# DanielPS555/Radix-sort-Merge-Sort-CUDA---Lab-y-practicos-GPGPU-2023

Measured on AMD Instinct MI355X. Metric: Mkeys/s sorting uint32, n=2^28, 1 GPU (+ merge-sort at 2/4/8), higher is better.
Workload: dtype u32; 1 GPU; LSD radix sort (8-bit digits, onesweep), n=2^28 uint32 u32, device-resident (BASELINE config 3); n_per_gpu=268435456, algo=radix, key=u32, dist=u32, parallelism=single GPU

## Files before the change

radix-sort-merge-sort-cuda---lab-y-practicos-gpgpu-2023_amd/csrc/fin_block.h:

```cpp
#pragma once
#include "segsort.h"

#include "devutil.h"

namespace labsort {

namespace {

#ifndef LABSORT_FIN_PREFETCH
#define LABSORT_FIN_PREFETCH 1
#endif

__device__ __forceinline__ uint32_t wave_incl_scan_dpp(uint32_t x) {
    x += (uint32_t)__builtin_amdgcn_update_dpp(0, (int)x, 0x111, 0xf, 0xf, false);
    x += (uint32_t)__builtin_amdgcn_update_dpp(0, (int)x, 0x112, 0xf, 0xf, false);
    x += (uint32_t)__builtin_amdgcn_update_dpp(0, (int)x, 0x114, 0xf, 0xf, false);
    x += (uint32_t)__builtin_amdgcn_update_dpp(0, (int)x, 0x118, 0xf, 0xf, false);
    x += (uint32_t)__builtin_amdgcn_update_dpp(0, (int)x, 0x142, 0xa, 0xf, false);
    x += (uint32_t)__builtin_amdgcn_update_dpp(0, (int)x, 0x143, 0xc, 0xf, false);
    return x;
}

template <int BLOCK, int KPT>
struct FinSmem {
    static constexpr int R = 256, W = BLOCK / WAVE, TILE = BLOCK * KPT;
    static_assert(TILE <= 65536, "16-bit LDS slots");
    static_assert(W == 4, "the fold holds one counter row per wave in registers");
    uint32_t keys[TILE];
    alignas(16) uint32_t cnt[W * R];
    alignas(16) uint32_t offs[W * R];
    uint32_t probe[WAVE];
    uint32_t ordered;
};

struct FinStripe {
    size_t sb;
    uint32_t ws0;
    uint32_t nf;
    uint32_t ng;
    bool tail_ok;
};
template <int W, int KPT>
__device__ __forceinline__ FinStripe fin_stripe(uint32_t b, uint32_t len, uint32_t lane, uint32_t wid) {
    if (len > (uint32_t)(W * WAVE * KPT)) len = 0u;
    const uint32_t jn = (len + (uint32_t)(W * WAVE) - 1u) / (uint32_t)(W * WAVE);
    const uint32_t ws0 = wid * jn * WAVE;
    const uint32_t rem = ws0 < len ? len - ws0 : 0u;
    const uint32_t nf = min(jn, rem / WAVE);
    const uint32_t tail = nf < jn ? rem - nf * WAVE : 0u;
    return {(size_t)b + ws0, ws0, nf, nf + (tail ? 1u : 0u), lane < tail};
}

template <int KPT>
__device__ __forceinline__ void fin_load(const uint32_t *in, const FinStripe &g, uint32_t lane, uint32_t (&k)[KPT]) {
    const char *pb = reinterpret_cast<const char *>(in + g.sb);
    const uint32_t lb = lane * 4u;
    if (g.nf == (uint32_t)KPT) {
#pragma unroll
        for (int j = 0; j < KPT; ++j) k[j] = ld_stream<NT_TILE>(reinterpret_cast<const uint32_t *>(pb + (lb + (uint32_t)(j * WAVE * 4))));
    } else {
#pragma unroll
        for (int j = 0; j < KPT; ++j) {
            k[j] = 0xFFFFFFFFu;
            if ((uint32_t)j < g.nf || ((uint32_t)j == g.nf && g.tail_ok))
                k[j] = ld_stream<NT_TILE>(reinterpret_cast<const uint32_t *>(pb + (lb + (uint32_t)(j * WAVE * 4))));
        }
    }
}

template <int BLOCK, int KPT>
__device__ __forceinline__ void fin_pass(FinSmem<BLOCK, KPT> &sm, const uint32_t (&k)[KPT], uint32_t shift, uint32_t ng,
                                         bool atomic_rank, uint32_t lane, uint32_t wid) {
    constexpr int W = FinSmem<BLOCK, KPT>::W, R = FinSmem<BLOCK, KPT>::R;
    uint32_t *wh = sm.cnt + wid * R;
    uint32_t *wo = sm.offs + wid * R;
    uint32_t n0 = ng, n1 = ng;
    asm volatile("" : "+s"(n0), "+s"(n1));
    uint32_t z = 0u;
    asm volatile("" : "+v"(z));
    *reinterpret_cast<uint4 *>(wh + 4u * lane) = make_uint4(z, z, z, z);
    uint32_t rank[KPT / 2] = {};
#pragma unroll
    for (int j = 0; j < KPT; ++j) {
        uint32_t r = 0u;
        if ((uint32_t)j < n0) r = rank8(wh, (k[j] >> shift) & 0xFFu, lane, atomic_rank);
        set16(rank, j, r);
    }
    __syncthreads();
    {
        uint4 c[W];
#pragma unroll
        for (int w = 0; w < W; ++w) c[w] = *reinterpret_cast<const uint4 *>(sm.cnt + w * R + 4u * lane);
        uint32_t tot[4] = {0u, 0u, 0u, 0u}, bef[4] = {0u, 0u, 0u, 0u};
#pragma unroll
        for (int w = 0; w < W; ++w) {
            const uint32_t cw[4] = {c[w].x, c[w].y, c[w].z, c[w].w};
            const bool before = (uint32_t)w < wid;
#pragma unroll
            for (int q = 0; q < 4; ++q) {
                tot[q] += cw[q];
                bef[q] += before ? cw[q] : 0u;
            }
        }
        const uint32_t s = tot[0] + tot[1] + tot[2] + tot[3];
        uint32_t run = wave_incl_scan_dpp(s) - s;
        uint4 o4;
        o4.x = run + bef[0];
        run += tot[0];
        o4.y = run + bef[1];
        run += tot[1];
        o4.z = run + bef[2];
        run += tot[2];
        o4.w = run + bef[3];
        *reinterpret_cast<uint4 *>(wo + 4u * lane) = o4;
    }
    __builtin_amdgcn_wave_barrier();
#pragma unroll
    for (int j = 0; j < KPT; ++j)
        if ((uint32_t)j < n1) set16(rank, j, wo[(k[j] >> shift) & 0xFFu] + get16(rank, j));
#pragma unroll
    for (int j = 0; j < KPT; ++j)
        if ((uint32_t)j < n1) sm.keys[get16(rank, j)] = k[j];
    __syncthreads();
}

template <int BLOCK, int KPT, int WPE>
__global__ __launch_bounds__(BLOCK, WPE) void k_fin_block(uint32_t *out, const uint32_t *__restrict__ off,
                                                           const uint32_t *__restrict__ hdr,
                                                           const uint32_t *__restrict__ list, HySel hy) {
    using S = FinSmem<BLOCK, KPT>;
    constexpr int W = S::W;
    constexpr int CLS = 3;
    constexpr bool PREFETCH = LABSORT_FIN_PREFETCH != 0;
    __shared__ S sm;
    if (hy.plan->hybrid == 0u) return;
    const uint32_t *in = hy.buf[hy.plan->fin_src];
    if (ld_agent(hdr) != 0u) return;
    const uint32_t cnt = hdr[SEG_HDR_CNT + CLS];
    const uint32_t tid = threadIdx.x, lane = tid & 63u, wid = __builtin_amdgcn_readfirstlane(tid >> 6);
    if (blockIdx.x >= cnt) return;
    probe_lane_order(sm.probe, &sm.ordered, lane, wid);
    __syncthreads();
    const bool atomic_rank = lane_order_probed(&sm.ordered);
    uint32_t nb, ne;
    {
        const uint32_t seg = __builtin_amdgcn_readfirstlane(list[blockIdx.x]);
        nb = __builtin_amdgcn_readfirstlane(off[seg]);
        ne = __builtin_amdgcn_readfirstlane(off[seg + 1]);
    }
    uint32_t k[KPT];
    FinStripe g = fin_stripe<W, KPT>(nb, ne - nb, lane, wid);
    if constexpr (PREFETCH) fin_load(in, g, lane, k);
    for (uint32_t it = blockIdx.x; it < cnt; it += gridDim.x) {
        if constexpr (!PREFETCH) {
            g = fin_stripe<W, KPT>(nb, ne - nb, lane, wid);
            fin_load(in, g, lane, k);
        }
        const bool more = it + gridDim.x < cnt;
        if (more) {
            const uint32_t seg = __builtin_amdgcn_readfirstlane(list[it + gridDim.x]);
            nb = __builtin_amdgcn_readfirstlane(off[seg]);
            ne = __builtin_amdgcn_readfirstlane(off[seg + 1]);
        }
        fin_pass(sm, k, 0u, g.ng, atomic_rank, lane, wid);
        {
            uint32_t n2 = g.ng;
            asm volatile("" : "+s"(n2));
#pragma unroll
            for (int j = 0; j < KPT; ++j)
                if ((uint32_t)j < n2) k[j] = sm.keys[g.ws0 + (uint32_t)j * WAVE + lane];
        }
        fin_pass(sm, k, 8u, g.ng, atomic_rank, lane, wid);
        FinStripe gn = g;
        uint32_t kn[PREFETCH ? KPT : 1];
        if constexpr (PREFETCH) {
            gn = fin_stripe<W, KPT>(nb, more ? ne - nb : 0u, lane, wid);
            fin_load(in, gn, lane, kn);
        }
        uint32_t nfs = g.nf;
        asm volatile("" : "+s"(nfs));
        const uint32_t *sk = sm.keys + g.ws0 + lane;
        char *ob = reinterpret_cast<char *>(out + g.sb);
        const uint32_t lb = lane * 4u;
        if (nfs == (uint32_t)KPT) {
#pragma unroll
            for (int j = 0; j < KPT; ++j) *reinterpret_cast<uint32_t *>(ob + (lb + (uint32_t)(j * WAVE * 4))) = sk[j * WAVE];
        } else {
#pragma unroll
            for (int j = 0; j < KPT; ++j)
                if ((uint32_t)j < nfs || ((uint32_t)j == nfs && g.tail_ok))
                    *reinterpret_cast<uint32_t *>(ob + (lb + (uint32_t)(j * WAVE * 4))) = sk[j * WAVE];
        }
        if constexpr (PREFETCH) {
            g = gn;
#pragma unroll
            for (int j = 0; j < KPT; ++j) k[j] = kn[j];
        }
    }
}

}

}
```

radix-sort-merge-sort-cuda---lab-y-practicos-gpgpu-2023_amd/csrc/kernels.hip:

```cpp
#include "common.h"
#include "devutil.h"
#include "host.h"
#include "lds_pass.h"

#include <cstdlib>
#include <cstring>
#include <type_traits>

namespace labsort {

__device__ __forceinline__ uint64_t mix64(uint64_t z) {
    z += 0x9E3779B97F4A7C15ull;
    z = (z ^ (z >> 30)) * 0xBF58476D1CE4E5B9ull;
    z = (z ^ (z >> 27)) * 0x94D049BB133111EBull;
    return z ^ (z >> 31);
}

__global__ __launch_bounds__(256) void k_fill(uint32_t *__restrict__ out, size_t n, uint64_t seed, int dist,
                                              uint64_t param, uint64_t first) {
    const size_t stride = (size_t)gridDim.x * blockDim.x;
    for (size_t i = (size_t)blockIdx.x * blockDim.x + threadIdx.x; i < n; i += stride) {
        const uint64_t gi = first + i;
        const uint64_t z = mix64(seed ^ (gi * 0x9E3779B97F4A7C15ull));
        const uint32_t hi = (uint32_t)(z >> 32);
// ... 162 lines not shown
                const bool s4 = fv(k[4 * u + 3]) == fa && fv(k[4 * u + 1]) == fa && fv(k[4 * u + 2]) == fa;
                if (s4) {
                    atomicAdd(ctr(fa), 4u);
                } else {
#pragma unroll
                    for (int j = 4 * u; j < 4 * u + 4; ++j) atomicAdd(ctr(fv(k[j])), 1u);
                }
            }
        };
        auto top = [&](uint32_t x) { return HY ? x >> (32 - HY_TOP_BITS) : fld(x, 2); };
        if (__ballot(top(k[0]) == top(k[3])) == 0ull) {
#pragma unroll
            for (int p = 0; p < NJ; ++p)
#pragma unroll
                for (int j = 0; j < 16; ++j) atomicAdd(&hj[p * JF + fld(k[j], p)], 1u);
            if constexpr (HY) {
#pragma unroll
                for (int j = 0; j < 16; ++j) atomicAdd(&ht[top(k[j])], 1u);
            }
            return;
        }
#pragma unroll
        for (int p = 0; p < NJ; ++p)
            add_field([&](uint32_t x) { return fld(x, p); }, [&](uint32_t f) { return &hj[p * JF + f]; });
        if constexpr (HY) add_field(top, [&](uint32_t f) { return &ht[f]; });
    };
    const uint32_t seg = blockIdx.x / bps, part = blockIdx.x % bps;
    const size_t sb = seg_start(seg, n), se = seg_start(seg + 1, n);
    const size_t per = (se - sb + bps - 1) / bps;
    const size_t beg = sb + (size_t)part * per < se ? sb + (size_t)part * per : se;
    const size_t end = beg + per < se ? beg + per : se;
    if ((((uintptr_t)keys) & 15u) == 0) {
        const size_t abeg = (beg + 3) & ~(size_t)3;
        const size_t vbeg = abeg < end ? abeg : end;
        for (size_t t = beg + threadIdx.x; t < vbeg; t += HIST_BLOCK) count(keys[t]);
        const size_t nv = (end - vbeg) / 4;
        const uint4 *v = reinterpret_cast<const uint4 *>(keys + vbeg);
        size_t i = threadIdx.x;
        uint4 c[4], x[4];
        if (i + 3 * HIST_BLOCK < nv) {
#pragma unroll
            for (int u = 0; u < 4; ++u) c[u] = ld_stream4<NT_HIST>(v + i + u * HIST_BLOCK);
        }
        for (; i + 3 * HIST_BLOCK < nv; i += 4 * HIST_BLOCK) {
            if (i + 7 * HIST_BLOCK < nv) {
#pragma unroll
                for (int u = 0; u < 4; ++u) x[u] = ld_stream4<NT_HIST>(v + i + (4 + u) * HIST_BLOCK);
            }
            count16(c);
#pragma unroll
            for (int u = 0; u < 4; ++u) c[u] = x[u];
        }
        for (; i < nv; i += HIST_BLOCK) {
            const uint4 x = ld_stream4<NT_HIST>(v + i);
            count(x.x); count(x.y); count(x.z); count(x.w);
        }
        for (size_t r = vbeg + nv * 4 + threadIdx.x; r < end; r += HIST_BLOCK) count(keys[r]);
    } else {
        for (size_t t = beg + threadIdx.x; t < end; t += HIST_BLOCK) count(keys[t]);
    }
    __syncthreads();
    for (int i = threadIdx.x; i < 256; i += HIST_BLOCK) {
        uint32_t c = 0;
#pragma unroll 8
        for (int q = 0; q < SL; ++q) c += h[i * SL + ((q + i) & (SL - 1))];
        if (c) atomicAdd(&hps[seg * 256 + i], c);
        if constexpr (HY) {
            uint32_t c2 = 0;
#pragma unroll
            for (int q = 0; q < 16; ++q) c2 += hj[JF + i * 16 + ((q + i) & 15)];
            if (c2) atomicAdd(&hy.hps2[seg * 256 + i], c2);
        }
    }
    const uint32_t rot = (blockIdx.x * (uint32_t)HIST_BLOCK) % ((uint32_t)NJ * JF);
    for (int i0 = threadIdx.x; i0 < NJ * JF; i0 += HIST_BLOCK) {
        int i = i0 + (int)rot;
        i = i >= NJ * JF ? i - NJ * JF : i;
        const uint32_t c = hj[i];
        const uint32_t p = (uint32_t)i / JF, f = (uint32_t)i % JF;
        if (c) atomicAdd(&joint[((p + 1) * NSEG + (f & 15u)) * 256 + (f >> 4)], c);
    }
    if constexpr (HY) {
        const uint32_t rot4 = (blockIdx.x * 272u) % (uint32_t)JF;
        for (uint32_t g0 = threadIdx.x; g0 < (uint32_t)JF; g0 += HIST_BLOCK) {
            const uint32_t f = (g0 + rot4) % (uint32_t)JF;
            uint32_t sum = 0;
#pragma unroll
            for (uint32_t q = 0; q < 4u; ++q) {
                const uint32_t c = ht[4u * f + q];
                sum += c;
                if (c) atomicAdd(&hy.top14[4u * f + q], c);
            }
            if (sum) atomicAdd(&joint[(3u * NSEG + (f & 15u)) * 256 + (f >> 4)], sum);
        }
    }
}

__device__ void build_segplan(SegPlan *__restrict__ sp, const uint32_t *__restrict__ hs, const uint32_t *start,
                              uint32_t mode, uint32_t *sh ) {
    const uint32_t t = threadIdx.x;
    uint32_t tot = 0;
    for (int s = 0; s < NSEG; ++s) {
        const uint32_t v = hs[s * 256 + t];
        sh[s * 256 + t] = v;
        tot += v;
    }
    uint32_t run = block_excl_scan<256, 256>(tot, sh + NSEG * 256);
    for (int s = 0; s < NSEG; ++s) {
        sp->base[s * 256 + t] = run;
        run += sh[s * 256 + t];
    }
    if (t <= (uint32_t)NSEG) sp->start[t] = start[t];
    if (t == 0) {
        uint32_t tp = 0, mx = 0;
        for (int s = 0; s <= NSEG; ++s) {
            sp->tpre[s] = tp;
            if (s < NSEG) {
                const uint32_t a0 = start[s] - start[s] % (uint32_t)OSP_TILE;
                const uint32_t ts = start[s + 1] > start[s] ? (start[s + 1] - a0 + OSP_TILE - 1) / OSP_TILE : 0u;
                tp += ts;
                mx = ts > mx ? ts : mx;
            }
        }
        sp->maxt = mx;
        sp->mode = mode;
        sp->segbits = mode == 2u ? 0u : 4u;
    }
}

__device__ void build_segplan_later(SegPlan *__restrict__ out, int q, uint32_t prev, uint32_t n, int seg_later,
                                    const uint32_t *hist, const uint32_t *__restrict__ joint, uint32_t *sh,
                                    uint32_t *start) {
    const uint32_t t = threadIdx.x;
    if (seg_later <= 0 || prev + 1u != (uint32_t)q) {
        for (int s = 0; s < NSEG; ++s) sh[s * 256 + t] = s ? 0u : hist[q * 256 + t];
        if (t <= (uint32_t)NSEG) start[t] = t ? n : 0u;
        __syncthreads();
        build_segplan(out, sh, start, 2u, sh);
        return;
    }
    const uint32_t ex = block_excl_scan<256, 256>(hist[prev * 256 + t], sh + NSEG * 256);
    if ((t & 15u) == 0) start[t >> 4] = ex;
    if (t == 0) start[NSEG] = n;
    __syncthreads();
    build_segplan(out, joint + (size_t)q * NSEG * 256, start, 1u, sh);
}

__global__ __launch_bounds__(256) void k_plan8(const uint32_t *__restrict__ hps, const uint32_t *__restrict__ joint,
                                               uint32_t n, int in_is_out, int seg_later, Plan *__restrict__ plan,
                                               SegPlan *__restrict__ sps, uint32_t *__restrict__ hist_out,
                                               uint4 *__restrict__ zp, size_t zn4, HyCounts hy) {
    constexpr uint32_t PW = 4;
    if (blockIdx.x >= PW) {
        const size_t stride = (size_t)(gridDim.x - PW) * blockDim.x;
        for (size_t i = (size_t)(blockIdx.x - PW) * blockDim.x + threadIdx.x; i < zn4; i += stride)
            zp[i] = make_uint4(0u, 0u, 0u, 0u);
        return;
    }
    const int me = (int)blockIdx.x;
    __shared__ uint32_t hist[4 * 256];
    __shared__ uint32_t sh[NSEG * 256 + 8];
    __shared__ uint32_t triv[4];
    __shared__ uint32_t start[NSEG + 1];
    __shared__ uint32_t prevs[4];
    __shared__ int first;
    __shared__ uint32_t max14;
    const uint32_t t = threadIdx.x;
    if (t < 4) triv[t] = 0;
    if (t == 0) max14 = 0u;
    __syncthreads();
    const uint32_t verdict = hy.ctl ? hy.ctl[HY_CTL_VERDICT] : 0u;
    if (hy.top14 && verdict == 0u) {
        uint32_t m = 0;
        for (uint32_t i = t; i < (uint32_t)HY_TOP; i += 256u) m = max(m, hy.top14[i]);
        atomicMax(&max14, m);
    }
    uint32_t v[4] = {0, 0, 0, 0};
    for (int s = 0; s < NSEG; ++s) {
        v[0] += hps[s * 256 + t];
#pragma unroll
        for (int p = 1; p < 4; ++p) v[p] += joint[(p * NSEG + s) * 256 + t];
    }
#pragma unroll
    for (int p = 0; p < 4; ++p) {
        hist[p * 256 + t] = v[p];
        if (me == 0) hist_out[p * 256 + t] = v[p];
        if (v[p] == n) triv[p] = 1;
    }
    if (t <= (uint32_t)NSEG) start[t] = seg_later < 0 ? (t ? n : 0u) : seg_start(t, n);
    __syncthreads();
    const bool hybrid = verdict ? verdict == HY_VERDICT_HYBRID
                                : hy.top14 && !triv[0] && !triv[1] && max14 <= min(hy.limit, HY_MAX_BUCKET);
    __syncthreads();
    if (hybrid && t < 2) triv[t] = 1;
    __syncthreads();
    if (t == 0 && me != 0) {
        int k = 0, last = -1;
        for (int p = 0; p < 4; ++p) {
            prevs[p] = NEXT_NONE;
            if (!triv[p]) {
                if (last >= 0) prevs[p] = (uint32_t)last;
                last = p;
                if (!k++) first = p;
            }
        }
        if (!k) first = -1;
    }
    if (t == 0 && me == 0) {
        int act[4];
        int k = 0;
        for (int p = 0; p < MAX_PASSES; ++p) {
            plan->src[p] = SEL_SKIP;
            plan->dst[p] = SEL_SKIP;
            plan->next[p] = NEXT_NONE;
            plan->prev[p] = NEXT_NONE;
        }
        for (int p = 0; p < 4; ++p) {
            prevs[p] = NEXT_NONE;
            if (!triv[p]) act[k++] = p;
        }
        for (int i = 0; i + 1 < k; ++i) {
            plan->next[act[i]] = (uint32_t)act[i + 1];
            plan->prev[act[i + 1]] = prevs[act[i + 1]] = (uint32_t)act[i];
        }
        plan->active = (uint32_t)k;
        first = k ? act[0] : -1;
        plan->hybrid = hybrid ? 1u : 0u;
        plan->fin_src = SEL_OUT;
        if (!hybrid) {
            plan_buffers(plan, act, k, in_is_out);
        } else {
            uint32_t src = SEL_IN;
            for (int i = 0; i < k; ++i) {
                plan->src[act[i]] = src;
                plan->dst[act[i]] = src = (i == k - 1 && !(k == 1 && in_is_out)) ? SEL_OUT : SEL_TMP;
            }
            plan->fin_src = src;
            plan->copy_from = SEL_SKIP;
        }
    }
    __syncthreads();
    if (first < 0 || me < first) return;
    if (me != first) {
        if (prevs[me] != NEXT_NONE)
            build_segplan_later(sps + me, me, prevs[me], n, seg_later, hist, joint, sh, start);
        return;
    }
    const uint32_t *hp = first == 0 ? hps : (hybrid && first == 2) ? hy.hps2 : nullptr;
    if (seg_later < 0 || !hp) {
        if (t <= (uint32_t)NSEG) start[t] = t ? n : 0u;
        for (int s = 0; s < NSEG; ++s) sh[s * 256 + t] = s ? 0u : hist[first * 256 + t];
        __syncthreads();
        build_segplan(sps + first, sh, start, 2u, sh);
    } else {
        for (int s = 0; s < NSEG; ++s) sh[s * 256 + t] = hp[s * 256 + t];
        __syncthreads();
        build_segplan(sps + first, sh, start, 0u, sh);
    }
}

__global__ __launch_bounds__(256) void k_final_copy(Bufs b, const Plan *__restrict__ plan, size_t n) {
    const uint32_t from = plan->copy_from;
    if (from == SEL_SKIP) return;
    const uint32_t *__restrict__ src = b.p[from];
    uint32_t *__restrict__ dst = b.p[SEL_OUT];
    const size_t stride = (size_t)gridDim.x * blockDim.x;
    const size_t tid = (size_t)blockIdx.x * blockDim.x + threadIdx.x;
    if (((((uintptr_t)src) | ((uintptr_t)dst)) & 15u) == 0) {
        const size_t nv = n / 4;
        for (size_t i = tid; i < nv; i += stride)
            reinterpret_cast<uint4 *>(dst)[i] = reinterpret_cast<const uint4 *>(src)[i];
        for (size_t i = nv * 4 + tid; i < n; i += stride) dst[i] = src[i];
    } else {
        for (size_t i = tid; i < n; i += stride) dst[i] = src[i];
    }
}

__device__ __forceinline__ uint32_t osp_pad(uint32_t i) { return i + (i >> 5); }

template <int BITS, int BLOCK, int KPT>
struct OsSmem {
    static constexpr int R = 1 << BITS, W = BLOCK / WAVE, TILE = BLOCK * KPT;
    uint32_t keys[TILE + TILE / 32];
    uint32_t whist[W * R];
    uint32_t gscan[R];
    uint32_t dstart[R];
    uint32_t delta[R];
    uint32_t wsum0[W];
    uint32_t wsum1[W];
    uint32_t tile;
};

template <int BITS, int BLOCK, int KPT>
__global__ __launch_bounds__(BLOCK) void k_onesweep(Bufs bufs, const Plan *__restrict__ plan, int pass, uint32_t n,
                                                    uint32_t flip, const uint32_t *__restrict__ ghist,
                                                    uint32_t *lookback, uint32_t *counter, uint32_t *err) {
    using S = OsSmem<BITS, BLOCK, KPT>;
    constexpr int R = S::R, W = S::W, TILE = S::TILE;
    constexpr uint32_t RM = R - 1;
    static_assert(R <= BLOCK, "one thread per digit");
    __shared__ S sm;

    const uint32_t srcsel = plan->src[pass];
    if (srcsel == SEL_SKIP) return;
    const uint32_t *__restrict__ in = bufs.p[srcsel];
    uint32_t *__restrict__ out = bufs.p[plan->dst[pass]];
    const uint32_t tid = threadIdx.x, lane = tid & 63u, wid = tid >> 6;
    const uint32_t shift = (uint32_t)pass * BITS;
// ... 1149 lines not shown
```

radix-sort-merge-sort-cuda---lab-y-practicos-gpgpu-2023_amd/csrc/segsort.hip:

```cpp
#include "segsort.h"

#include <algorithm>

#include "devutil.h"
#include "fin_block.h"
#include "host.h"
#include "seg_kernels.h"

namespace labsort {

namespace {

constexpr int BIN_BLOCK = 1024, BIN_SPT = 4;

__global__ __launch_bounds__(BIN_BLOCK) void k_seg_bin(const uint32_t *__restrict__ off, uint32_t nseg, uint32_t n,
                                                        uint32_t max_len, SegEdges e, uint32_t copy1,
                                                        uint32_t *__restrict__ hdr, uint32_t *__restrict__ lists,
                                                        size_t stride, const Plan *__restrict__ hyplan) {
    __shared__ uint32_t cnt[SEG_CLASSES], base[SEG_CLASSES];
    if (hyplan && hyplan->hybrid == 0u) return;
    const uint32_t tid = threadIdx.x, lane = tid & 63u;
    if (tid < (uint32_t)SEG_CLASSES) cnt[tid] = 0u;
    __syncthreads();
    uint32_t cls[BIN_SPT], pos[BIN_SPT];
    bool bad = false;
#pragma unroll
    for (int j = 0; j < BIN_SPT; ++j) {
        const uint32_t seg = blockIdx.x * (uint32_t)(BIN_BLOCK * BIN_SPT) + (uint32_t)j * BIN_BLOCK + tid;
        uint32_t c = SEG_CLASSES;
        if (seg < nseg) {
            const uint32_t a = off[seg], b = off[seg + 1];
            if (b < a || b > n) {
                bad = true;
            } else {
                const uint32_t len = b - a;
                if (max_len && len > max_len) bad = true;
                if (len > 1u || (len == 1u && copy1)) {
                    c = 0u;
#pragma unroll
                    for (int q = 0; q < SEG_CLASSES - 1; ++q) c += len > e.e[q] ? 1u : 0u;
                }
            }
            if (seg == 0u && a != 0u) bad = true;
            if (seg == nseg - 1u && b != n) bad = true;
        }
        cls[j] = c;
        pos[j] = 0u;
        if (lists) {
#pragma unroll
            for (uint32_t cc = 0; cc < (uint32_t)SEG_CLASSES; ++cc) {
                const uint64_t m = __ballot(c == cc);
                if (m == 0ull) continue;
                const uint32_t leader = (uint32_t)__ffsll((long long)m) - 1u;
                uint32_t wb = 0u;
                if (lane == leader) wb = atomicAdd(&cnt[cc], (uint32_t)__popcll(m));
                wb = __shfl(wb, (int)leader);
                if (c == cc) pos[j] = wb + mbcnt64(m);
            }
        }
    }
    if (bad) atomicOr(hdr, 1u);
    if (!lists) return;
    __syncthreads();
    if (tid < (uint32_t)SEG_CLASSES) base[tid] = cnt[tid] ? atomicAdd(hdr + SEG_HDR_CNT + tid, cnt[tid]) : 0u;
    __syncthreads();
#pragma unroll
    for (int j = 0; j < BIN_SPT; ++j) {
        const uint32_t seg = blockIdx.x * (uint32_t)(BIN_BLOCK * BIN_SPT) + (uint32_t)j * BIN_BLOCK + tid;
        if (cls[j] < (uint32_t)SEG_CLASSES) lists[(size_t)cls[j] * stride + base[cls[j]] + pos[j]] = seg;
    }
}

__global__ __launch_bounds__(256) void k_seg_ids(const uint32_t *__restrict__ off, uint32_t nseg, uint32_t n,
                                                 const uint32_t *__restrict__ idx, uint32_t *__restrict__ ids,
                                                 uint32_t *__restrict__ iota, const uint32_t *__restrict__ hdr) {
    if (ld_agent(hdr) != 0u) return;
    const size_t stride = (size_t)gridDim.x * blockDim.x;
    for (size_t i = (size_t)blockIdx.x * blockDim.x + threadIdx.x; i < n; i += stride) {
        if (iota) iota[i] = (uint32_t)i;
        if (!ids) continue;
        uint32_t p = idx ? idx[i] : (uint32_t)i;
        if (p >= n) p = n - 1u;
        uint32_t lo = 1u, hi = nseg;
        while (lo < hi) {
            const uint32_t mid = lo + (hi - lo) / 2u;
            if (off[mid] > p) hi = mid;
            else lo = mid + 1u;
        }
        ids[i] = lo - 1u;
    }
}

__global__ __launch_bounds__(256) void k_seg_gather(const uint32_t *__restrict__ src, const uint32_t *__restrict__ vsrc,
                                                    const uint32_t *__restrict__ perm, uint32_t *__restrict__ out,
                                                    uint32_t *__restrict__ vout, uint32_t n,
                                                    const uint32_t *__restrict__ hdr) {
    if (ld_agent(hdr) != 0u) return;
    const size_t stride = (size_t)gridDim.x * blockDim.x;
    for (size_t i = (size_t)blockIdx.x * blockDim.x + threadIdx.x; i < n; i += stride) {
        uint32_t p = perm ? perm[i] : (uint32_t)i;
        if (p >= n) p = n - 1u;
        out[i] = src[p];
        if (vsrc) vout[i] = vsrc[p];
    }
}

__global__ void k_seg_err_acc(uint32_t *hdr, uint32_t *inner) {
    if (threadIdx.x == 0 && blockIdx.x == 0) {
        if (*inner) hdr[SEG_HDR_DEVERR] = 1u;
        *inner = 0u;
    }
}

unsigned stream_blocks(size_t n) {
    size_t b = (n + 256 * 8 - 1) / (256 * 8);
    return (unsigned)(b < 1 ? 1 : b > 8192 ? 8192 : b);
}

hipError_t launch_seg_sort(int c, const uint32_t *in, uint32_t *out, const uint32_t *vin, uint32_t *vout,
                           const uint32_t *off, const uint32_t *hdr, const uint32_t *list, uint32_t flip,
                           hipStream_t s, const HySel &hy = HySel{}, bool f32 = false) {
    return f32 ? launch_seg_sort_f32(c, in, out, vin, vout, off, hdr, list, flip, s, hy)
               : launch_seg_sort_t<false>(c, in, out, vin, vout, off, hdr, list, flip, s, hy);
}

hipError_t launch_seg_ids(const uint32_t *off, size_t nseg, size_t n, const uint32_t *idx, uint32_t *ids,
                          uint32_t *iota, const uint32_t *hdr, hipStream_t s) {
    k_seg_ids<<<stream_blocks(n), 256, 0, s>>>(off, (uint32_t)nseg, (uint32_t)n, idx, ids, iota, hdr);
    return hipGetLastError();
}

hipError_t launch_seg_gather(const uint32_t *src, const uint32_t *vsrc, const uint32_t *perm, uint32_t *out,
                             uint32_t *vout, size_t n, const uint32_t *hdr, hipStream_t s) {
    k_seg_gather<<<stream_blocks(n), 256, 0, s>>>(src, vsrc, perm, out, vout, (uint32_t)n, hdr);
    return hipGetLastError();
}

hipError_t launch_seg_err_acc(uint32_t *hdr, uint32_t *inner_err, hipStream_t s) {
    k_seg_err_acc<<<1, 64, 0, s>>>(hdr, inner_err);
    return hipGetLastError();
}

}

hipError_t launch_seg_bin(const uint32_t *off, size_t nseg, size_t n, size_t max_len, bool pairs, bool copy1,
                          uint32_t *hdr, uint32_t *lists, size_t stride, hipStream_t s) {
    const unsigned g = (unsigned)((nseg + BIN_BLOCK * BIN_SPT - 1) / (BIN_BLOCK * BIN_SPT));
    (void)pairs;
    const SegEdges e{{(uint32_t)SEG_WAVE_KEYS, (uint32_t)SEG_WAVE2_KEYS, (uint32_t)SEG_WAVE3_KEYS, (uint32_t)SEG_BLOCK_KEYS}};
    k_seg_bin<<<g, BIN_BLOCK, 0, s>>>(off, (uint32_t)nseg, (uint32_t)n, (uint32_t)max_len, e, copy1 ? 1u : 0u, hdr, lists,
                                      stride, nullptr);
    return hipGetLastError();
}

hipError_t launch_seg_lds_classes(size_t max_len, bool pairs, const uint32_t *in, uint32_t *out, const uint32_t *vin,
                                  uint32_t *vout, const uint32_t *off, const uint32_t *hdr, const uint32_t *lists,
                                  size_t stride, uint32_t flip, bool f32, hipStream_t s) {
    (void)pairs;
    for (int c = 0; c <= seg_class_of(max_len); ++c) {
        const hipError_t e = launch_seg_sort(c, in, out, vin, vout, off, hdr, lists + (size_t)c * stride, flip, s, HySel{}, f32);
        if (e != hipSuccess) return e;
    }
    return hipSuccess;
}

namespace {
constexpr int FE_BLOCK = 1024, FE_W = FE_BLOCK / WAVE, FE_KPT = OSP_TILE / FE_BLOCK;
static_assert(FE_KPT * FE_BLOCK == OSP_TILE && HY_BUCKETS == 256u * 256u, "one tile per boundary, one workgroup per digit-2 value");

__device__ uint32_t fin_edge_at(uint32_t P, const uint32_t *__restrict__ keys, uint32_t flip, const SegPlan *__restrict__ sp,
                                const uint32_t *__restrict__ lb, uint32_t nslots, uint32_t *wh, bool &bad) {
    const uint32_t tid = threadIdx.x, wid = tid >> 6;
    uint32_t sg = 0;
    for (uint32_t s = 1; s < (uint32_t)NSEG; ++s) sg = sp->start[s] <= P ? s : sg;
    const uint32_t s0 = sp->start[sg], a0 = s0 - s0 % (uint32_t)OSP_TILE;
    const uint32_t l = (P - a0) / (uint32_t)OSP_TILE, beg = l ? a0 + l * (uint32_t)OSP_TILE : s0;
    for (uint32_t i = tid; i < (uint32_t)(FE_W * 256); i += FE_BLOCK) wh[i] = 0u;
    uint32_t k[FE_KPT];
#pragma unroll
    for (int j = 0; j < FE_KPT; ++j) {
        const uint32_t i = beg + (uint32_t)j * FE_BLOCK + tid;
        k[j] = i < P ? keys[i] : 0u;
    }
    __syncthreads();
#pragma unroll
    for (int j = 0; j < FE_KPT; ++j)
        if (beg + (uint32_t)j * FE_BLOCK + tid < P) atomicAdd(&wh[wid * 256u + ((k[j] ^ flip) >> 24)], 1u);
    __syncthreads();
    if (tid >= 256u) return 0u;
    uint32_t r = sp->base[sg * 256u + tid];
#pragma unroll
    for (int w = 0; w < FE_W; ++w) r += wh[(uint32_t)w * 256u + tid];
    if (l) {
        const uint32_t slot = sp->tpre[sg] + l - 1u;
        const uint32_t w = slot < nslots ? lb[(size_t)slot * 256u + tid] : 0u;
        if ((w & LB_INC) == 0u) bad = true;
        r += w & LB_VAL;
    }
    return r;
}

__global__ __launch_bounds__(FE_BLOCK) void k_fin_edges(const Plan *__restrict__ plan, Bufs bufs, uint32_t n, uint32_t flip,
                                                        const uint32_t *__restrict__ hist, const SegPlan *__restrict__ sp,
                                                        const uint32_t *__restrict__ lb, uint32_t nslots, uint32_t *err,
                                                        uint32_t *hdr, uint32_t *__restrict__ off) {
    __shared__ uint32_t wh[FE_W * 256];
    __shared__ uint32_t wsum[4];
    __shared__ uint32_t s2;
    if (plan->hybrid == 0u) return;
    const uint32_t tid = threadIdx.x, d2 = blockIdx.x;
    const uint32_t h2 = tid < 256u ? hist[2 * 256 + tid] : 0u;
    const uint32_t x2 = block_excl_scan<FE_BLOCK, 256>(h2, wsum);
    if (tid == d2) s2 = min(x2, n);
    __syncthreads();
    const uint32_t P = s2;
    uint32_t o;
    bool bad = false;
    if (plan->src[3] == SEL_SKIP) {
        const uint32_t h3 = tid < 256u ? hist[3 * 256 + tid] : 0u;
        o = block_excl_scan<FE_BLOCK, 256>(h3, wsum) + (h3 == n ? P : 0u);
    } else {
        o = fin_edge_at(P, bufs.p[plan->src[3]], flip, sp, lb, nslots, wh, bad);
    }
    if (tid >= 256u) return;
    if (bad) {
        atomicOr(err, 1u);
        atomicOr(hdr, 1u);
        return;
    }
    const uint32_t q = (tid << 8) | d2;
    off[q] = o;
    if (q == HY_BUCKETS - 1u) off[HY_BUCKETS] = n;
}
}

hipError_t launch_hybrid_finish(const Plan *plan, Bufs b, size_t n, uint32_t flip, const uint32_t *hist, const SegPlan *sp3,
                                const uint32_t *lookback3, size_t nslots, uint32_t *err, uint32_t *hdr, uint32_t *off,
                                uint32_t *lists, hipStream_t s) {
    const size_t stride = HY_BUCKETS;
    k_fin_edges<<<256, FE_BLOCK, 0, s>>>(plan, b, (uint32_t)n, flip, hist, sp3, lookback3, (uint32_t)nslots, err, hdr, off);
    hipError_t e = hipGetLastError();
    if (e != hipSuccess) return e;
    const SegEdges ed{{(uint32_t)SEG_WAVE_KEYS, (uint32_t)SEG_WAVE2_KEYS, (uint32_t)SEG_WAVE3_KEYS, (uint32_t)HY_BLOCK_KEYS}};
    k_seg_bin<<<HY_BUCKETS / (BIN_BLOCK * BIN_SPT), BIN_BLOCK, 0, s>>>(off, HY_BUCKETS, (uint32_t)n, HY_MAX_BUCKET, ed, 1u, hdr,
                                                                      lists, stride, plan);
    if ((e = hipGetLastError()) != hipSuccess) return e;
    const HySel hy{plan, {b.p[0], b.p[1], b.p[2]}};
    uint32_t *out = b.p[SEL_OUT];
    const unsigned cus = (unsigned)cu_count();
    for (int c = 0; c < SEG_CLASSES; ++c) {
        const uint32_t *list = lists + (size_t)c * stride;
        if (c == 3) {
            k_fin_block<HY_BLOCK, HY_BLOCK_KPT, HY_BLOCK_WPE><<<cus * (unsigned)HY_BLOCK_WPE, HY_BLOCK, 0, s>>>(out, off, hdr, list, hy);
            e = hipGetLastError();
        } else {
            e = launch_seg_sort(c, out, out, nullptr, nullptr, off, hdr, list, flip, s, hy);
        }
        if (e != hipSuccess) return e;
    }
    return hipSuccess;
}

size_t seg_inner_bytes(size_t n) {
    const size_t m = n < (size_t)LABSORT_AUTO_PAIRS_MERGE_MAX_KEYS ? n : (size_t)LABSORT_AUTO_PAIRS_MERGE_MAX_KEYS;
    return std::max(labsort_pairs_workspace_bytes(n, LABSORT_ALGO_AUTO), labsort_pairs_workspace_bytes(m, LABSORT_ALGO_MERGE));
}

}

using namespace labsort;

extern "C" {

size_t labsort_segment_tile_keys(void) { return (size_t)SEG_TILE_KEYS; }
size_t labsort_segment_pair_tile_keys(void) { return (size_t)SEG_TILE_PAIRS; }

int labsort_segment_class_edges(int pairs, size_t *edges, int cap) {
    const size_t e[SEG_CLASSES] = {(size_t)SEG_WAVE_KEYS, (size_t)SEG_WAVE2_KEYS, (size_t)SEG_WAVE3_KEYS, (size_t)SEG_BLOCK_KEYS,
                                   pairs ? (size_t)SEG_TILE_PAIRS : (size_t)SEG_TILE_KEYS};
    for (int i = 0; i < SEG_CLASSES && i < cap && edges; ++i) edges[i] = e[i];
    return SEG_CLASSES;
}

namespace {
bool seg_lds_path(size_t max_len, int pairs) {
    return max_len > 0 && max_len <= (pairs ? (size_t)SEG_TILE_PAIRS : (size_t)SEG_TILE_KEYS);
}
struct SegLayout {
    size_t off_lists, list_stride;
    size_t off_a, off_b, off_c, off_inner, inner_bytes;
    size_t total;
};
SegLayout seg_layout(size_t n, size_t nseg, bool lds) {
    SegLayout L{};
    Carver c{SEG_HDR_BYTES};
    if (lds) {
        L.list_stride = align_up(nseg * 4, 256) / 4;
        L.off_lists = c.take((size_t)SEG_CLASSES * L.list_stride * 4);
        L.total = c.o;
    } else {
        L.off_a = c.take(n * 4);
        L.off_b = c.take(n * 4);
        L.off_c = c.take(n * 4);
        L.off_inner = c.o;
        L.inner_bytes = seg_inner_bytes(n);
        L.total = c.o + L.inner_bytes;
    }
    return L;
}

int sort_segments(const uint32_t *ki, const uint32_t *vi, uint32_t *ko, uint32_t *vo, size_t n, const uint32_t *off,
                  size_t nseg, size_t max_len, int key_type, void *d_ws, size_t ws_bytes, void *stream) {
    const bool pairs = vi != nullptr || vo != nullptr;
    if (n == 0) return LABSORT_OK;
    if (!ki || !ko || !off || (pairs && (!vi || !vo))) return LABSORT_ERR_ARG;
    if (!device_key_type_ok(key_type)) return LABSORT_ERR_ARG;
    if (nseg == 0 || n > (size_t)0x7FFFFFFFu || nseg > (size_t)0x7FFFFFFFu) return LABSORT_ERR_ARG;
    if (pairs && !pairs_alias_ok(ki, vi, ko, vo)) return LABSORT_ERR_ARG;
    const bool lds = seg_lds_path(max_len, pairs ? 1 : 0);
    if (!lds && n > RADIX_MAX_N) return LABSORT_ERR_ARG;
    if (!d_ws || ws_bytes < labsort_segments_workspace_bytes(n, nseg, max_len, pairs ? 1 : 0)) return LABSORT_ERR_ARG;
    const SegLayout L = seg_layout(n, nseg, lds);
    const uint32_t flip = flip_of(key_type);
    hipStream_t s = as_stream(stream);
    char *ws = static_cast<char *>(d_ws);
    uint32_t *hdr = reinterpret_cast<uint32_t *>(ws);
    const bool inplace = ki == ko;
    HIP_TRY(launch_zero(hdr, SEG_HDR_BYTES, s));
    if (lds) {
        uint32_t *lists = reinterpret_cast<uint32_t *>(ws + L.off_lists);
        TimingScope ts(LABSORT_K_SEGSORT, s);
        HIP_TRY(launch_seg_bin(off, nseg, n, max_len, pairs, !inplace, hdr, lists, L.list_stride, s));
        HIP_TRY(launch_seg_lds_classes(max_len, pairs, ki, ko, vi, vo, off, hdr, lists, L.list_stride, flip,
                                       key_type == LABSORT_KEY_F32, s));
        return LABSORT_OK;
    }
    uint32_t *A = reinterpret_cast<uint32_t *>(ws + L.off_a), *B = reinterpret_cast<uint32_t *>(ws + L.off_b),
             *C = reinterpret_cast<uint32_t *>(ws + L.off_c);
    char *iws = ws + L.off_inner;
    uint32_t *ierr = reinterpret_cast<uint32_t *>(iws);
    HIP_TRY(launch_zero(ierr, 16, s));
    {
        TimingScope ts(LABSORT_K_SEGSORT, s);
        HIP_TRY(launch_seg_bin(off, nseg, n, max_len, pairs, false, hdr, nullptr, 0, s));
        if (pairs) HIP_TRY(launch_seg_ids(off, nseg, n, nullptr, nullptr, A, hdr, s));
        else HIP_TRY(launch_seg_ids(off, nseg, n, nullptr, A, nullptr, hdr, s));
    }
    int st;
    if ((st = labsort_sort_pairs_device(ki, A, B, C, n, key_type, LABSORT_ALGO_AUTO, iws, L.inner_bytes, stream))) return st;
    HIP_TRY(launch_seg_err_acc(hdr, ierr, s));
    if (pairs) {
        {
            TimingScope ts(LABSORT_K_SEGSORT, s);
            HIP_TRY(launch_seg_ids(off, nseg, n, C, B, nullptr, hdr, s));
        }
        if ((st = labsort_sort_pairs_device(B, C, B, C, n, LABSORT_KEY_U32, LABSORT_ALGO_AUTO, iws, L.inner_bytes, stream)))
            return st;
        HIP_TRY(launch_seg_err_acc(hdr, ierr, s));
        TimingScope ts(LABSORT_K_SEGSORT, s);
        if (inplace) {
            HIP_TRY(launch_seg_gather(ki, vi, C, A, B, n, hdr, s));
            HIP_TRY(launch_seg_gather(A, B, nullptr, ko, vo, n, hdr, s));
        } else {
            HIP_TRY(launch_seg_gather(ki, vi, C, ko, vo, n, hdr, s));
        }
    } else {
        if ((st = labsort_sort_pairs_device(C, B, C, B, n, LABSORT_KEY_U32, LABSORT_ALGO_AUTO, iws, L.inner_bytes, stream)))
            return st;
        HIP_TRY(launch_seg_err_acc(hdr, ierr, s));
        TimingScope ts(LABSORT_K_SEGSORT, s);
        HIP_TRY(launch_seg_gather(B, nullptr, nullptr, ko, nullptr, n, hdr, s));
    }
    return LABSORT_OK;
}
}

size_t labsort_segments_workspace_bytes(size_t n, size_t nseg, size_t max_segment_keys, int pairs) {
    return seg_layout(n, nseg, seg_lds_path(max_segment_keys, pairs)).total;
}

int labsort_sort_segments_device(const void *d_keys_in, void *d_keys_out, size_t n, const uint32_t *d_offsets,
                                 size_t nseg, size_t max_segment_keys, int key_type, void *d_ws, size_t ws_bytes,
                                 void *stream) {
    return sort_segments(static_cast<const uint32_t *>(d_keys_in), nullptr, static_cast<uint32_t *>(d_keys_out), nullptr,
                         n, d_offsets, nseg, max_segment_keys, key_type, d_ws, ws_bytes, stream);
}

int labsort_sort_segments_pairs_device(const void *d_keys_in, const void *d_vals_in, void *d_keys_out, void *d_vals_out,
                                       size_t n, const uint32_t *d_offsets, size_t nseg, size_t max_segment_keys,
                                       int key_type, void *d_ws, size_t ws_bytes, void *stream) {
    if (n == 0) return LABSORT_OK;
    if (!d_vals_in || !d_vals_out) return LABSORT_ERR_ARG;
    return sort_segments(static_cast<const uint32_t *>(d_keys_in), static_cast<const uint32_t *>(d_vals_in),
                         static_cast<uint32_t *>(d_keys_out), static_cast<uint32_t *>(d_vals_out), n, d_offsets, nseg,
                         max_segment_keys, key_type, d_ws, ws_bytes, stream);
}

int labsort_segments_workspace_status(const void *d_ws, void *stream) {
    uint32_t w[2] = {0, 0};
    if (const int st = read_ws_words(d_ws, w, 2, as_stream(stream))) return st;
    return w[0] ? LABSORT_ERR_ARG : w[SEG_HDR_DEVERR] ? LABSORT_ERR_DEVICE : LABSORT_OK;
}

}
```

Measured before the change: 149,200 Mkeys/s.

## Fold bucket binning into the block finish kernel and drop the per-class launches

The hybrid finish no longer runs a binning kernel followed by four class-specific segment-sort launches. The block-level finish kernel now walks the 65536 buckets itself in a grid-stride loop, sorts every non-empty bucket that fits one tile, and appends oversized buckets to a list that a single class-4 segment-sort launch then handles. Separately, the zeroing kernel skips the first half of its region when the hybrid verdict is set. This cuts launch count and the binning pass, but small buckets now use full 1024-thread block passes instead of wave-level sorters, and every workgroup scans empty buckets serially.

```diff
diff --git a/harness/fin_small_buckets.py b/harness/fin_small_buckets.py
--- /dev/null
+++ b/harness/fin_small_buckets.py
@@ -0,0 +1,82 @@
+#!/usr/bin/env python3
+import argparse
+import ctypes
+import os
+import sys
+
+import torch
+
+from finish_ab import ALGO_RADIX, K_SEGSORT, fmt, load, ls
+
+
+def small_bucket_keys(n, seed):
+    g = torch.Generator(device="cuda")
+    g.manual_seed(seed)
+    r = torch.randint(0, 1 << 32, (n,), dtype=torch.int64, device="cuda", generator=g)
+    sel = torch.randint(0, 64, (n,), dtype=torch.int64, device="cuda", generator=g)
+    r = (r & ~(3 << 16)) | (torch.clamp(sel, max=3) << 16)
+    del sel
+    return torch.where(r >= (1 << 31), r - (1 << 32), r).to(torch.int32)
+
+
+def main():
+    ap = argparse.ArgumentParser()
+    ap.add_argument("--lib", action="append", default=[], help="NAME=PATH; empty PATH: the package's library")
+    ap.add_argument("--reps", type=int, default=9)
+    ap.add_argument("--warmup", type=int, default=2)
+    ap.add_argument("--out", default="")
+    a = ap.parse_args()
+    if not torch.cuda.is_available():
+        sys.exit("fin_small_buckets: no GPU (no CPU fallback)")
+    out = open(a.out, "a") if a.out else sys.stdout
+    os.environ.pop("LABSORT_RADIX_HYBRID", None)
+    builds = {}
+    for spec in a.lib or ["this="]:
+        name, _, path = spec.partition("=")
+        builds[name] = load(path)
+    st = torch.cuda.current_stream().cuda_stream
+    n = 1 << 28
+    keys = small_bucket_keys(n, 0x5EED0003)
+    torch.cuda.empty_cache()
+    res = torch.empty_like(keys)
+    nbytes = max(int(lib.labsort_workspace_bytes(n, ALGO_RADIX)) for lib in builds.values())
+    ws = torch.zeros(nbytes, dtype=torch.uint8, device="cuda")
+    first = None
+    fin = {k: [] for k in builds}
+    tot = {k: [] for k in builds}
+    for rep in range(a.warmup + a.reps):
+        for name, lib in builds.items():
+            lib.labsort_timing_enable(1)
+            e0, e1 = torch.cuda.Event(enable_timing=True), torch.cuda.Event(enable_timing=True)
+            e0.record()
+            rc = lib.labsort_sort_device(keys.data_ptr(), res.data_ptr(), n, 0, ALGO_RADIX, ws.data_ptr(), nbytes, st)
+            e1.record()
+            e1.synchronize()
+            if rc or lib.labsort_workspace_status(ws.data_ptr(), n, ALGO_RADIX, st):
+                sys.exit(f"fin_small_buckets: {name}: the sort failed")
+            ms, cnt = ctypes.c_double(0.0), ctypes.c_longlong(0)
+            lib.labsort_timing_read(K_SEGSORT, ctypes.byref(ms), ctypes.byref(cnt))
+            lib.labsort_timing_enable(0)
+            if rep == 0:
+                if int(lib.labsort_radix_path(ws.data_ptr(), n, st)) != 1:
+                    sys.exit(f"fin_small_buckets: {name}: the input did not take the hybrid path")
+                if first is None:
+                    first = res.clone()
+                    u = first ^ -(1 << 31)
+                    if not bool((u[1:] >= u[:-1]).all()):
+                        sys.exit(f"fin_small_buckets: {name}: the result is not sorted")
+                    del u
+                elif not torch.equal(res, first):
+                    sys.exit(f"fin_small_buckets: {name}: result differs from the first build's")
+            if rep >= a.warmup:
+                fin[name].append(ms.value)
+                tot[name].append(e0.elapsed_time(e1))
+    print(f"# 2^28 keys, three buckets of ~256 keys and one of ~15600 in every top-14-bit group: {torch.cuda.get_device_name(0)}; "
+          f"{a.reps} alternating repetitions after {a.warmup} warm-ups; ms per sort, median [min, max]", file=out)
+    for name in builds:
+        print(f"{name:>8}  finish {fmt(fin[name])}   whole sort (timing hooks on) {fmt(tot[name])}", file=out)
+    out.flush()
+
+
+if __name__ == "__main__":
+    main()
diff --git a/radix-sort-merge-sort-cuda---lab-y-practicos-gpgpu-2023_amd/csrc/fin_block.h b/radix-sort-merge-sort-cuda---lab-y-practicos-gpgpu-2023_amd/csrc/fin_block.h
--- a/radix-sort-merge-sort-cuda---lab-y-practicos-gpgpu-2023_amd/csrc/fin_block.h
+++ b/radix-sort-merge-sort-cuda---lab-y-practicos-gpgpu-2023_amd/csrc/fin_block.h
@@ -124,43 +124,60 @@
     __syncthreads();
 }
 
+constexpr uint32_t FIN_BAD = 0xFFFFFFFFu;
+
+__device__ __forceinline__ uint32_t fin_next(uint32_t &q, uint32_t &nb, uint32_t ne, uint32_t step, uint32_t n, uint32_t max_here,
+                                             const uint32_t *__restrict__ off, uint32_t *hdr, uint32_t *list4) {
+    while (q < HY_BUCKETS) {
+        const uint32_t len = ne - nb;
+        if (ne < nb || ne > n || len > HY_MAX_BUCKET) {
+            if (threadIdx.x == 0u) atomicOr(hdr, 1u);
+            return FIN_BAD;
+        }
+        if (len != 0u && len <= max_here) return len;
+        if (len != 0u && threadIdx.x == 0u) list4[atomicAdd(hdr + SEG_HDR_CNT + 4, 1u)] = q;
+        q += step;
+        if (q < HY_BUCKETS) {
+            nb = __builtin_amdgcn_readfirstlane(off[q]);
+            ne = __builtin_amdgcn_readfirstlane(off[q + 1]);
+        }
+    }
+    return 0u;
+}
+
 template <int BLOCK, int KPT, int WPE>
-__global__ __launch_bounds__(BLOCK, WPE) void k_fin_block(uint32_t *out, const uint32_t *__restrict__ off,
-                                                           const uint32_t *__restrict__ hdr,
-                                                           const uint32_t *__restrict__ list, HySel hy) {
+__global__ __launch_bounds__(BLOCK, WPE) void k_fin_block(uint32_t *out, const uint32_t *__restrict__ off, uint32_t n,
+                                                           uint32_t *hdr, uint32_t *list4, HySel hy) {
     using S = FinSmem<BLOCK, KPT>;
     constexpr int W = S::W;
-    constexpr int CLS = 3;
     constexpr bool PREFETCH = LABSORT_FIN_PREFETCH != 0;
     __shared__ S sm;
     if (hy.plan->hybrid == 0u) return;
     const uint32_t *in = hy.buf[hy.plan->fin_src];
     if (ld_agent(hdr) != 0u) return;
-    const uint32_t cnt = hdr[SEG_HDR_CNT + CLS];
     const uint32_t tid = threadIdx.x, lane = tid & 63u, wid = __builtin_amdgcn_readfirstlane(tid >> 6);
-    if (blockIdx.x >= cnt) return;
+    uint32_t q = blockIdx.x, nb = 0u, ne = 0u;
+    if (q < HY_BUCKETS) {
+        nb = __builtin_amdgcn_readfirstlane(off[q]);
+        ne = __builtin_amdgcn_readfirstlane(off[q + 1]);
+    }
+    uint32_t len = __builtin_amdgcn_readfirstlane(fin_next(q, nb, ne, gridDim.x, n, (uint32_t)S::TILE, off, hdr, list4));
+    if (len == 0u || len == FIN_BAD) return;
     probe_lane_order(sm.probe, &sm.ordered, lane, wid);
     __syncthreads();
     const bool atomic_rank = lane_order_probed(&sm.ordered);
-    uint32_t nb, ne;
-    {
-        const uint32_t seg = __builtin_amdgcn_readfirstlane(list[blockIdx.x]);
-        nb = __builtin_amdgcn_readfirstlane(off[seg]);
-        ne = __builtin_amdgcn_readfirstlane(off[seg + 1]);
-    }
     uint32_t k[KPT];
-    FinStripe g = fin_stripe<W, KPT>(nb, ne - nb, lane, wid);
+    FinStripe g = fin_stripe<W, KPT>(nb, len, lane, wid);
     if constexpr (PREFETCH) fin_load(in, g, lane, k);
-    for (uint32_t it = blockIdx.x; it < cnt; it += gridDim.x) {
+    for (;;) {
         if constexpr (!PREFETCH) {
-            g = fin_stripe<W, KPT>(nb, ne - nb, lane, wid);
+            g = fin_stripe<W, KPT>(nb, len, lane, wid);
             fin_load(in, g, lane, k);
         }
-        const bool more = it + gridDim.x < cnt;
-        if (more) {
-            const uint32_t seg = __builtin_amdgcn_readfirstlane(list[it + gridDim.x]);
-            nb = __builtin_amdgcn_readfirstlane(off[seg]);
-            ne = __builtin_amdgcn_readfirstlane(off[seg + 1]);
+        q += gridDim.x;
+        if (q < HY_BUCKETS) {
+            nb = __builtin_amdgcn_readfirstlane(off[q]);
+            ne = __builtin_amdgcn_readfirstlane(off[q + 1]);
         }
         fin_pass(sm, k, 0u, g.ng, atomic_rank, lane, wid);
         {
@@ -171,10 +188,12 @@
                 if ((uint32_t)j < n2) k[j] = sm.keys[g.ws0 + (uint32_t)j * WAVE + lane];
         }
         fin_pass(sm, k, 8u, g.ng, atomic_rank, lane, wid);
+        len = __builtin_amdgcn_readfirstlane(fin_next(q, nb, ne, gridDim.x, n, (uint32_t)S::TILE, off, hdr, list4));
+        if (len == FIN_BAD) return;
         FinStripe gn = g;
         uint32_t kn[PREFETCH ? KPT : 1];
         if constexpr (PREFETCH) {
-            gn = fin_stripe<W, KPT>(nb, more ? ne - nb : 0u, lane, wid);
+            gn = fin_stripe<W, KPT>(nb, len, lane, wid);
             fin_load(in, gn, lane, kn);
         }
         uint32_t nfs = g.nf;
@@ -191,6 +210,7 @@
                 if ((uint32_t)j < nfs || ((uint32_t)j == nfs && g.tail_ok))
                     *reinterpret_cast<uint32_t *>(ob + (lb + (uint32_t)(j * WAVE * 4))) = sk[j * WAVE];
         }
+        if (len == 0u) break;
         if constexpr (PREFETCH) {
             g = gn;
 #pragma unroll
diff --git a/radix-sort-merge-sort-cuda---lab-y-practicos-gpgpu-2023_amd/csrc/kernels.hip b/radix-sort-merge-sort-cuda---lab-y-practicos-gpgpu-2023_amd/csrc/kernels.hip
--- a/radix-sort-merge-sort-cuda---lab-y-practicos-gpgpu-2023_amd/csrc/kernels.hip
+++ b/radix-sort-merge-sort-cuda---lab-y-practicos-gpgpu-2023_amd/csrc/kernels.hip
@@ -338,8 +338,9 @@
                                                uint4 *__restrict__ zp, size_t zn4, HyCounts hy) {
     constexpr uint32_t PW = 4;
     if (blockIdx.x >= PW) {
+        const size_t z0 = hy.ctl && hy.ctl[HY_CTL_VERDICT] == HY_VERDICT_HYBRID ? zn4 / 4 * 2 : 0;
         const size_t stride = (size_t)(gridDim.x - PW) * blockDim.x;
-        for (size_t i = (size_t)(blockIdx.x - PW) * blockDim.x + threadIdx.x; i < zn4; i += stride)
+        for (size_t i = z0 + (size_t)(blockIdx.x - PW) * blockDim.x + threadIdx.x; i < zn4; i += stride)
             zp[i] = make_uint4(0u, 0u, 0u, 0u);
         return;
     }
diff --git a/radix-sort-merge-sort-cuda---lab-y-practicos-gpgpu-2023_amd/csrc/segsort.hip b/radix-sort-merge-sort-cuda---lab-y-practicos-gpgpu-2023_amd/csrc/segsort.hip
--- a/radix-sort-merge-sort-cuda---lab-y-practicos-gpgpu-2023_amd/csrc/segsort.hip
+++ b/radix-sort-merge-sort-cuda---lab-y-practicos-gpgpu-2023_amd/csrc/segsort.hip
@@ -16,9 +16,8 @@
 __global__ __launch_bounds__(BIN_BLOCK) void k_seg_bin(const uint32_t *__restrict__ off, uint32_t nseg, uint32_t n,
                                                         uint32_t max_len, SegEdges e, uint32_t copy1,
                                                         uint32_t *__restrict__ hdr, uint32_t *__restrict__ lists,
-                                                        size_t stride, const Plan *__restrict__ hyplan) {
+                                                        size_t stride) {
     __shared__ uint32_t cnt[SEG_CLASSES], base[SEG_CLASSES];
-    if (hyplan && hyplan->hybrid == 0u) return;
     const uint32_t tid = threadIdx.x, lane = tid & 63u;
     if (tid < (uint32_t)SEG_CLASSES) cnt[tid] = 0u;
     __syncthreads();
@@ -149,7 +148,7 @@
     (void)pairs;
     const SegEdges e{{(uint32_t)SEG_WAVE_KEYS, (uint32_t)SEG_WAVE2_KEYS, (uint32_t)SEG_WAVE3_KEYS, (uint32_t)SEG_BLOCK_KEYS}};
     k_seg_bin<<<g, BIN_BLOCK, 0, s>>>(off, (uint32_t)nseg, (uint32_t)n, (uint32_t)max_len, e, copy1 ? 1u : 0u, hdr, lists,
-                                      stride, nullptr);
+                                      stride);
     return hipGetLastError();
 }
 
@@ -241,24 +240,13 @@
     k_fin_edges<<<256, FE_BLOCK, 0, s>>>(plan, b, (uint32_t)n, flip, hist, sp3, lookback3, (uint32_t)nslots, err, hdr, off);
     hipError_t e = hipGetLastError();
     if (e != hipSuccess) return e;
-    const SegEdges ed{{(uint32_t)SEG_WAVE_KEYS, (uint32_t)SEG_WAVE2_KEYS, (uint32_t)SEG_WAVE3_KEYS, (uint32_t)HY_BLOCK_KEYS}};
-    k_seg_bin<<<HY_BUCKETS / (BIN_BLOCK * BIN_SPT), BIN_BLOCK, 0, s>>>(off, HY_BUCKETS, (uint32_t)n, HY_MAX_BUCKET, ed, 1u, hdr,
-                                                                      lists, stride, plan);
-    if ((e = hipGetLastError()) != hipSuccess) return e;
     const HySel hy{plan, {b.p[0], b.p[1], b.p[2]}};
     uint32_t *out = b.p[SEL_OUT];
-    const unsigned cus = (unsigned)cu_count();
-    for (int c = 0; c < SEG_CLASSES; ++c) {
-        const uint32_t *list = lists + (size_t)c * stride;
-        if (c == 3) {
-            k_fin_block<HY_BLOCK, HY_BLOCK_KPT, HY_BLOCK_WPE><<<cus * (unsigned)HY_BLOCK_WPE, HY_BLOCK, 0, s>>>(out, off, hdr, list, hy);
-            e = hipGetLastError();
-        } else {
-            e = launch_seg_sort(c, out, out, nullptr, nullptr, off, hdr, list, flip, s, hy);
-        }
-        if (e != hipSuccess) return e;
-    }
-    return hipSuccess;
+    uint32_t *list4 = lists + (size_t)4 * stride;
+    const unsigned grid = std::min((unsigned)cu_count() * (unsigned)HY_BLOCK_WPE, (unsigned)HY_BUCKETS);
+    k_fin_block<HY_BLOCK, HY_BLOCK_KPT, HY_BLOCK_WPE><<<grid, HY_BLOCK, 0, s>>>(out, off, (uint32_t)n, hdr, list4, hy);
+    if ((e = hipGetLastError()) != hipSuccess) return e;
+    return launch_seg_sort(4, out, out, nullptr, nullptr, off, hdr, list4, flip, s, hy);
 }
 
 size_t seg_inner_bytes(size_t n) {
```

Result: no change. 150,200 Mkeys/s, median of 6 (+0.7%).
